# smilne36/ComponentFrameworks-smoothed-particle-hydrodynamics

Measured on AMD Instinct MI355X. Metric: particle-substeps/sec, higher is better.
Workload: dtype f32; 1 GPU; config3: 4194304 particles and a 128x128x128-cell grid per GPU (BASELINE.json configs[2]); particles=4194304, neighbor_kernel=k_sph_walk

## Files before the change

componentframeworks-smoothed-particle-hydrodynamics_amd/csrc/sph_engine.hip:

```cpp
#include <hip/hip_runtime.h>

#include <algorithm>
#include <chrono>
#include <cstdarg>
#include <cstdio>
#include <cstdlib>
#include <cstring>
#include <memory>
#include <mutex>
#include <set>
#include <string>
#include <thread>
#include <vector>

#include "../../include/sph_abi.h"
#include "sph_host.h"
#include "sph_kernels.h"
#include "sph_walk.h"
#include "sph_sample.h"
#include "sph_neighbors.h"
#include "sph_components.h"
#include "sph_knn.h"
#include "sph_aggregate.h"
#include "sph_conv.h"
// ... 177 lines not shown
    size_t cap = 0;
    int allocatedCells = 0;
    uint32_t idBase = 0;

    int optNeighbor = 3, optGridBuild = 0, optAos = 1, optTiming = 0, optGraph = 0;
    struct GraphEntry {
        uint64_t key = 0;
        std::vector<unsigned char> material;
        hipGraphExec_t exec = nullptr;
        int postCur = 0;
        bool postAos = false, postAcc = false;
        uint64_t lastUse = 0;
    };
    std::vector<GraphEntry> graphs;
    uint64_t graphClock = 0, graphLaunches = 0, graphCaptures = 0;

    SphParticle* d_aos = nullptr;
    float4* d_pos[2] = {nullptr, nullptr};
    float4* d_vel[2] = {nullptr, nullptr};
    float2* d_rp[2] = {nullptr, nullptr};
    float* d_foam[2] = {nullptr, nullptr};
    float4* d_acc = nullptr;
    int cur = 0;
    bool internalValid = false, aosValid = false, accValid = false;
    uint2* d_binKey = nullptr;
    uint32_t* d_order = nullptr;
    float4* d_stencil = nullptr;
    size_t stencilCount = 0;
    int32_t *d_llNext = nullptr, *d_llCell = nullptr, *d_llKey = nullptr;
    uint2* d_tmp = nullptr;
    uint32_t *d_cellCount = nullptr, *d_cellStart = nullptr, *d_blockSums = nullptr;
    int32_t* d_dbg = nullptr;
    size_t dbgCap = 0;
    bool slab = false;
    int z0 = 0, z1 = 0, hasLo = 0, hasHi = 0;
    size_t nSlots = 0;
    char* d_face[4] = {nullptr, nullptr, nullptr, nullptr};
    SlabSeen* h_seen = nullptr;
    hipEvent_t evCnt[4] = {nullptr, nullptr, nullptr, nullptr};
    bool cntValid[4] = {false, false, false, false};
    uint32_t exchangeNo = 0;
    sph::SlabMsg msgSend{}, msgRecv{};
    uint64_t sentBytes[2] = {0, 0};
    int calmHold = 0;
    uint32_t stepNo = 0;
    SphSlabIntent intent{};
    bool intentValid = false;
    uint32_t holdEvents = 0;
    int verifyMode = 1;
    double deadlineSec = 30.0;
    float lastDt = 0.0f;
    int tightMessages = 0;
    hipStream_t hstream = nullptr;
    hipEvent_t evIntent = nullptr;
    SlabPlans *d_intent = nullptr, *h_intent = nullptr;
    float handshakeMs = 0.0f;
    uint64_t handshakes = 0;
    bool stepPaused = false;
    float packGrid[8] = {0};
    bool packGridValid = false;
    hipEvent_t evX[5] = {nullptr, nullptr, nullptr, nullptr, nullptr};
    hipEvent_t evPassEnd = nullptr;
    uint32_t faceCap = 0;
    const void* faceAgreedWith = nullptr;
    SphFountain fountain{};
    SphRiver river{};
    std::vector<float> terrainHeights;
    float* d_terrain = nullptr;
    size_t terrainCap = 0;
    float4 *d_sPV = nullptr, *d_sOwn = nullptr;
    size_t sortedCap = 0;
    float4* d_shapeTab = nullptr;
    float shapeKey[8] = {-1.0f};
    sph::ShapeTab shapeTab{};
    hipStream_t xstream = nullptr;
    hipStream_t bstream = nullptr;
    hipEvent_t evBoundary = nullptr, evPacked = nullptr, evDone = nullptr, evSorted = nullptr, evInterior = nullptr;
    hipEvent_t peerDone[2] = {nullptr, nullptr};
    bool stepPending = false;
    bool slabOrderValid = false;
    float lastContainer[15] = {0};
    uint32_t* d_slabCnt = nullptr;
    int debugFlags = 0;
    unsigned long long* d_stats = nullptr;
    DevBuf<float4> d_sampleIn;
    DevBuf<SphSample> d_sampleOut;
    DevBuf<int32_t> d_slotIds;
    ScanScratch scanScratch;
    DevBuf<int32_t> d_nbIndices;
    DevBuf<uint32_t> d_nbCnt;
    DevBuf<long long> d_nbOffsets;
    SphNeighborInfo nbInfo{};
    bool nbIndexed = false;
    DevBuf<int32_t> d_ccIds, d_ccLabels, d_ccRoots;
    DevBuf<uint32_t> d_ccParent, d_ccMinId, d_ccFlag, d_ccWords;
    DevBuf<unsigned long long> d_ccStats;
    DevBuf<long long> d_ccOffsets;
    DevBuf<sph::CcRow> d_ccTable;
    SphComponentInfo ccInfo{};
    bool ccValid = false;
    int optCcVariant = 0;
    DevBuf<int32_t> d_knnIndices;
    DevBuf<float> d_knnDist2;
    DevBuf<uint32_t> d_knnCounts;
    DevBuf<unsigned long long> d_knnStats;
    SphKnnInfo knnInfo{};
    DevBuf<float4> d_rayIn, d_rayHits;
    DevBuf<unsigned long long> d_rayStats;
    DevBuf<uint2> d_rayBin;
    DevBuf<uint32_t> d_rayCount, d_rayStart, d_rayBlockSums, d_rayOrder;
    int optRaysVariant = 0;
    SphRaysInfo raysInfo{};
    bool raysValid = false;
    DevBuf<uint4> d_spanRows;
    DevBuf<unsigned long long> d_spanStats;
    int optRaySpansVariant = 0;
    SphRaySpansInfo spansInfo{};
    bool spansValid = false;
    int optKnnVariant = 0;
    DevBuf<float> d_aggStage, d_aggIn, d_aggOut;
    DevBuf<uint32_t> d_aggCnt;
    DevBuf<uint2> d_adjKey;
    DevBuf<uint32_t> d_adjCount, d_adjSums, d_adjStart, d_adjTmp, d_adjPerm, d_adjArg;
    DevBuf<float4> d_adjPts;
    DevBuf<float> d_adjIn;
    DevBuf<float> d_posStage;
    int optAggVariant = 0;
    DevBuf<sph::ShellRow> d_shRows;
    DevBuf<int32_t> d_shIds, d_shSlots;
    DevBuf<float4> d_shNrm;
    DevBuf<uint32_t> d_shFlagRow, d_shFlagSlot;
    DevBuf<unsigned long long> d_shStats;
    DevBuf<long long> d_shOffsets;
    SphShellInfo shellInfo{};
    DevBuf<sph::AnisoRow> d_anRows;
    DevBuf<float4> d_anSlots;
    DevBuf<unsigned long long> d_anStats;
    SphAnisoInfo anisoInfo{};
    int optShellTimed = 0;
    DevBuf<float> d_surfVol;
    DevBuf<uint16_t> d_surfCode;
    DevBuf<uint32_t> d_surfVOff, d_surfTris;
    DevBuf<uint2> d_surfTile;
    DevBuf<unsigned long long> d_surfTileOff;
    DevBuf<sph::SurfVertex> d_surfVerts;
    bool surfValid = false;
    uint32_t surfNumV = 0, surfNumT = 0;
    DevBuf<double> d_statSums;
    DevBuf<uint32_t> d_statPart, d_statHist;
    DevBuf<unsigned long long> d_statCell, d_statOut;

    float4* d_trRec = nullptr;
    uint32_t* d_trPerm = nullptr;
    float4* d_trRing = nullptr;
    uint32_t* d_trState = nullptr;
    uint2* d_trKey = nullptr;
    DevBuf<uint32_t> d_trCellCount, d_trCellStart, d_trBlockSums;
    size_t trM = 0, trCap = 0, trRingCap = 0;
    int trIntegrator = 0;
    uint32_t trK = 0, trS = 1;
    uint64_t trSteps = 0;
    uint64_t trSorted = 0;
    bool trOrdered = false;
    bool capturing = false;

    float4* d_dfPool = nullptr;
// ... 836 lines not shown
                          p.param_shapeAux[0], p.param_shapeAux[1], p.param_shapeAux[2], 1.0f};
    if (e->d_shapeTab && std::memcmp(key, e->shapeKey, sizeof(key)) == 0) return SPH_OK;
    int rc;
    if (!e->d_shapeTab && (rc = dev_alloc(&e->d_shapeTab, 128))) return rc;
    float pts[384], b0[3];
    const int cnt = shape_table(p, pts, b0);
    float4 host[128];
    for (int i = 0; i < cnt; ++i) host[i] = make_float4(pts[3 * i], pts[3 * i + 1], pts[3 * i + 2], 0.0f);
    if (cnt) {
        HIP_TRY(hipStreamSynchronize(e->stream));
        HIP_TRY(hipMemcpy(e->d_shapeTab, host, sizeof(float4) * (size_t)cnt, hipMemcpyHostToDevice));
    }
    e->shapeTab = sph::ShapeTab{e->d_shapeTab, cnt, b0[0], b0[1], b0[2]};
    std::memcpy(e->shapeKey, key, sizeof(key));
    return SPH_OK;
}

int dispatch_one(SphEngine* e, float overrideDt, bool boundaryFirst = false) {
    if (e->params.param_pause) { if (boundaryFirst) HIP_TRY(hipEventRecord(e->evBoundary, e->stream)); return SPH_OK; }
    int rc;
    if (e->trM && (rc = needs_sorted_copy(e, "tracers need"))) return rc;
    if (e->scK && (rc = needs_sorted_copy(e, "scalars need"))) return rc;
    if (e->dfC && (rc = needs_sorted_copy(e, "diffuse particles need"))) return rc;
    if (e->gtTab.count && (rc = needs_sorted_copy(e, "gates need"))) return rc;
    if (e->monCount && (rc = needs_sorted_copy(e, "monitors need"))) return rc;
    if ((rc = validate_params(e->params)) || (rc = couple_refused(e))) return rc;
    float cont[15];
    container_key(e->params, cont);
    const bool sameContainer = std::memcmp(cont, e->lastContainer, sizeof(cont)) == 0;
    const float dt = overrideDt > 0.0f ? overrideDt : e->params.param_timeStep;
    e->lastDt = dt;
    compute_grid_extents(e->params, e->grid);
    if ((rc = ensure_grid_buffers(e))) return rc;
    SimK k;
    make_simk(e->params, e->grid, dt, k);
    if (e->dfC && e->dfCrOn) {
        float radius = 0.0f;
        int stencil = 0;
        if (!diffuse_crest_args(e, k.cellSize, &radius, &stencil))
            return fail(SPH_ERR_STATE, "diffuse crest radius %g is above three cells (%g) of this grid", (double)radius, (double)(3.0f * k.cellSize));
    }
    if (e->slab) {
        if (e->z1 > e->grid.dims[2] || e->z0 < 0) return fail(SPH_ERR_STATE, "slab [%d,%d) outside the %d-layer grid", e->z0, e->z1, e->grid.dims[2]);
        k.gz = e->z1 - e->z0 + 2; k.numCells = k.gx * k.gy * k.gz; k.zoff = e->z0 - 1;
        if (e->optGridBuild != 1 && sameContainer) k.slabFlags = e->d_slabCnt + kSlabCntFlags;
    }
    if ((rc = import_state(e))) return rc;
    const int n = (int)(e->slab ? e->nSlots : e->n);
    StateIn in{e->d_pos[e->cur], e->d_vel[e->cur], e->d_rp[e->cur], e->d_foam[e->cur]};
    const int nx = e->cur ^ 1;
    if (k.obbDeferred && (rc = ensure_shape_table(e))) return rc;
    const bool fuseAos = !e->slab && e->optAos == 0 && e->aosValid && !k.obbDeferred && !e->obsK && !e->cpBuoy;
    StateOut out{e->d_pos[nx], e->d_vel[nx], e->d_rp[nx], e->d_foam[nx], e->d_acc, fuseAos ? e->d_aos : nullptr, e->idBase};
    if (e->optGridBuild == 1) {
        if (e->slab) return fail(SPH_ERR_STATE, "the linked-list variant is single-GPU only");
        if (!e->d_llNext) {
            if ((rc = dev_alloc(&e->d_llNext, e->cap)) || (rc = dev_alloc(&e->d_llCell, e->cap)) || (rc = dev_alloc(&e->d_llKey, e->cap))) return rc;
        }
        int32_t* cellHead = reinterpret_cast<int32_t*>(e->d_cellStart);
        {
            Timed t(e, SPH_K_SCAN);
            hipLaunchKernelGGL(k_ll_clear, dim3(blocks_for((size_t)k.numCells)), dim3(kBlock), 0, e->stream, cellHead, k.numCells);
        }
        if (n) {
            {
                Timed t(e, SPH_K_BIN);
                hipLaunchKernelGGL(k_ll_build, dim3(blocks_for(n)), dim3(kBlock), 0, e->stream, k, in.pos, cellHead, e->d_llNext, e->d_llCell, e->d_llKey, n);
            }
            Timed t(e, SPH_K_SPH);
            hipLaunchKernelGGL(k_sph_ll, dim3(blocks_for(n)), dim3(kBlock), 0, e->stream, k, in, out, cellHead, e->d_llNext, n);
        }
    } else {
    if ((rc = build_grid(e, k, true))) return rc;
    if (e->trM && (rc = tracers_advect(e, k, dt))) return rc;
    if (e->monCount && (rc = monitors_step(e, k, dt))) return rc;
    if (e->dfC && (rc = diffuse_step(e, k, dt, (uint32_t)n))) return rc;
    if (e->scK && (rc = scalars_step(e, k, dt))) return rc;
    if (n) {
        if (!e->d_sPV || e->sortedCap < (size_t)n) return fail(SPH_ERR_STATE, "sorted copy missing");
        const uint32_t* live = e->slab ? e->d_cellStart + k.numCells : nullptr;
        SortedIn S{e->d_sPV, e->d_sOwn};
        Timed t(e, SPH_K_SPH);
        if (e->optNeighbor >= 3 && (size_t)n < ((size_t)1 << 27)) {
            const dim3 grid(8 * ((blocks_for(n, 256) + 7) / 8));
            auto walk = [&](hipStream_t st, const uint32_t* lo, const uint32_t* hi, bool bothEnds = false) {
                const int dbg = (e->debugFlags & ~256) | (bothEnds ? 256 : 0);
                if (k.h2 <= 1.0f)
                    hipLaunchKernelGGL((k_sph_walk<SPH_WALK_MAXN, SPH_WALK_UNROLL, SPH_WALK_CAP, true>), grid, dim3(256), 0, st, k, S, in, out,
                                       e->d_order, e->d_cellStart, live, n, dbg, e->d_stats, lo, hi);
                else
                    hipLaunchKernelGGL((k_sph_walk<SPH_WALK_MAXN, SPH_WALK_UNROLL, SPH_WALK_CAP, false>), grid, dim3(256), 0, st, k, S, in, out,
                                       e->d_order, e->d_cellStart, live, n, dbg, e->d_stats, lo, hi);
            };
            const bool split = boundaryFirst && e->slab && k.gz > 2 * kSlabDepth && !k.obbDeferred && sameContainer;
            const bool timedStep = boundaryFirst && e->optTiming && e->evPassEnd;
            if (split) {
                const uint32_t* endLo = e->d_cellStart + kSlabDepth * (size_t)(k.gx * k.gy);
                const uint32_t* startHi = e->d_cellStart + (size_t)(k.gz - kSlabDepth) * (size_t)(k.gx * k.gy);
                HIP_TRY(hipEventRecord(e->evSorted, e->stream));
                walk(e->stream, endLo, startHi, true);
                HIP_TRY(hipEventRecord(e->evBoundary, e->stream));
                HIP_TRY(hipStreamWaitEvent(e->bstream, e->evSorted, 0));
                walk(e->bstream, endLo, startHi);
                HIP_TRY(hipEventRecord(e->evInterior, e->bstream));
                boundaryFirst = false;
                HIP_TRY(hipStreamWaitEvent(e->stream, e->evInterior, 0));
            } else {
                walk(e->stream, nullptr, nullptr);
            }
            if (timedStep) HIP_TRY(hipEventRecord(e->evPassEnd, e->stream));
        } else if (e->optNeighbor >= 2) {
            hipLaunchKernelGGL((k_sph_list<SPH_LIST_MAXN, SPH_LIST_UNROLL, SPH_LIST_CAP>), dim3(8 * ((blocks_for(n, SPH_LIST_BLOCK) + 7) / 8)), dim3(SPH_LIST_BLOCK), 0, e->stream, k, S, in, out,
                               e->d_order, e->d_cellStart, live, n, e->debugFlags, e->d_stats);
        } else {
            hipLaunchKernelGGL(k_sph_slow, dim3(blocks_for(n)), dim3(kBlock), 0, e->stream, k, S, in, out, e->d_order, e->d_cellStart, n);
        }
    }
    }
    if (n && k.obbDeferred) {
        Timed t(e, SPH_K_OTHER);
        const uint32_t* live = (e->slab && e->optGridBuild != 1) ? e->d_cellStart + k.numCells : nullptr;
        hipLaunchKernelGGL(k_obb_ext, dim3(blocks_for(n)), dim3(kBlock), 0, e->stream, k, e->shapeTab, out.pos, out.vel, live, n,
                           (e->slab && e->optGridBuild != 1) ? (const float4*)e->d_sOwn : (const float4*)nullptr);
    }
    if (e->obsK && (rc = obstacles_step(e, out.pos, out.vel, n, dt))) return rc;
    if (e->scK && (e->cpBuoy || e->cpTab.nSrc) && (rc = couple_step(e, out.pos, out.vel, n, dt))) return rc;
    if (e->gtTab.count && (rc = gates_step(e, out.pos, out.vel, n, dt))) return rc;
    const bool riverOn = e->river.riverMode && !e->terrainHeights.empty();
    if (riverOn) {
        if (e->slab) return fail(SPH_ERR_STATE, "riverMode on a z-slab engine: recycled particles jump across slabs (single-GPU engines only)");
        if (n) {
            const SphParams& p = e->params;
            const SphRiver& r = e->river;
            RiverK rk{r.terrainW, r.terrainH, r.terrainWorldMinX, r.terrainWorldMinZ, r.terrainWorldSizeX, r.terrainWorldSizeZ,
                      0.02f, 1.0f - 0.05f, p.param_boxCenter[0], r.riverAmp, r.riverFreq, r.riverPhase, r.riverChannelWidth,
                      80.0f, p.param_timeStep, r.riverSinkY, r.riverSinkZMax, r.riverEmitterPos[0], r.riverEmitterPos[1], r.riverEmitterPos[2],
                      r.riverEmitterVel[0], r.riverEmitterVel[1], r.riverEmitterVel[2], r.riverEmitterRadius,
                      r.riverSinkZMax - r.riverEmitterPos[2], p.param_restDensity};
            Timed t(e, SPH_K_OTHER);
            hipLaunchKernelGGL(k_river, dim3(blocks_for(n)), dim3(kBlock), 0, e->stream, rk, e->d_terrain, out.pos, out.vel, out.rp,
                               fuseAos ? (float4*)nullptr : e->d_acc, fuseAos ? e->d_aos : (SphParticle*)nullptr, e->d_aos, e->idBase, n);
        }
    }
    if (e->fountain.fountainMode && !e->river.riverMode) {
        if (e->slab) return fail(SPH_ERR_STATE, "fountainMode on a z-slab engine: recycled particles jump across slabs (single-GPU engines only)");
        if (n) {
            float half[3];
            effective_half(e->params, half);
            const SphParams& p = e->params;
            const SphFountain& f = e->fountain;
            FountainK fk{p.param_boxCenter[0] + f.fountainOffset[0], p.param_boxCenter[1] + f.fountainOffset[1],
                         p.param_boxCenter[2] + f.fountainOffset[2], f.fountainRadius, f.fountainSpread, f.fountainJetSpeedLive,
                         (p.param_boxCenter[1] - half[1]) + f.fountainDrainLevel, std::fmin(1.0f, f.fountainDrainPerSec * dt),
                         p.param_restDensity, f.fountainSeed * 747796405u};
            Timed t(e, SPH_K_OTHER);
            const uint32_t* live = (e->slab && e->optGridBuild != 1) ? e->d_cellStart + k.numCells : nullptr;
            hipLaunchKernelGGL(k_fountain, dim3(blocks_for(n)), dim3(kBlock), 0, e->stream, fk, out.pos, out.vel, out.rp,
                               fuseAos ? (float4*)nullptr : e->d_acc, fuseAos ? e->d_aos : (SphParticle*)nullptr, e->idBase, live, n);
        }
        e->fountain.fountainSeed++;
    }
    HIP_TRY(hipGetLastError());
    if (boundaryFirst) HIP_TRY(hipEventRecord(e->evBoundary, e->stream));
    e->cur = nx;
    e->accValid = !fuseAos;
    e->aosValid = fuseAos;
    if (e->slab) {
        const bool sorted = e->optGridBuild != 1 && n > 0;
        if (!sorted) HIP_TRY(hipMemcpyAsync(e->d_slabCnt + kSlabCntLive, e->d_cellStart + k.numCells, sizeof(uint32_t), hipMemcpyDeviceToDevice, e->stream));
        if (!sameContainer) slab_hold(e);
        std::memcpy(e->lastContainer, cont, sizeof(cont));
        e->slabOrderValid = sorted && sameContainer;
        return SPH_OK;
    }
    if (e->optAos == 0 && !e->aosValid) return writeback(e);
// ... 9 lines not shown
    sph::compute_grid_extents(e->params, e->grid);
    SlabGeom g;
    g.gminz = e->grid.gridMin[2]; g.cellSize = e->grid.cellSize; g.gzGlobal = e->grid.dims[2];
    g.z0 = e->z0; g.z1 = e->z1; g.hasLo = e->hasLo; g.hasHi = e->hasHi;
    return g;
}

int slab_engine(const SphEngine* e, bool needFaces = false) {
    if (!e) return fail(SPH_ERR_ARG, "null engine");
    if (needFaces) return e->slab && e->d_face[0] ? SPH_OK : fail(SPH_ERR_STATE, "slab engine with face buffers required");
    return e->slab ? SPH_OK : fail(SPH_ERR_STATE, "not a slab engine");
}

int slab_flags_error(const SphEngine* e, uint32_t flags, uint32_t nLo, uint32_t nHi) {
    if (flags & SPH_SLAB_FLAG_SEND_OVERFLOW) return fail(SPH_ERR_CAPACITY, "halo send buffer overflowed (%u / %u records for a capacity of %u)", nLo, nHi, e->faceCap);
    if (flags & SPH_SLAB_FLAG_SLOT_OVERFLOW) return fail(SPH_ERR_CAPACITY, "slab capacity %zu exceeded while appending halo records", e->cap);
    if (flags & SPH_SLAB_FLAG_BAD_HEADER) return fail(SPH_ERR_HIP, "a received halo message did not start with a valid header (magic / count): failed or garbled receive");
    if (flags & SPH_SLAB_FLAG_TRUNCATED) return fail(SPH_ERR_CAPACITY, "a neighbour rank had more halo records than its message could carry (face capacity %u)", e->faceCap);
    if (flags & SPH_SLAB_FLAG_SIZE_MISMATCH) return fail(SPH_ERR_STATE, "the two ends of a link sized an exchange's messages differently (a received header names other message sizes than this engine received): "
                                                "the ranks' call sequences differ");
    return SPH_OK;
}

template <class K>
int launch_impulse(SphEngine* e, const K& kk) {
    int rc;
    if ((rc = import_state(e))) return rc;
    const size_t nw = e->slab ? e->nSlots : e->n;
    if (e->slab) slab_hold(e);
    if (nw) {
        Timed t(e, SPH_K_IMPULSE);
        hipLaunchKernelGGL((k_impulse<K>), dim3(blocks_for(nw)), dim3(kBlock), 0, e->stream, kk, e->d_pos[e->cur], e->d_vel[e->cur],
                           (e->aosValid && !e->slab) ? e->d_aos : nullptr, e->idBase, (int)nw);
    }
    HIP_TRY(hipGetLastError());
    return SPH_OK;
}
}

extern "C" {

int sph_abi_version(void) { return SPH_ABI_VERSION; }
const char* sph_last_error(void) { return g_err.c_str(); }

int sph_params_default(SphParams* out) {
    if (!out) return fail(SPH_ERR_ARG, "null params");
    sph::params_default(*out);
    return SPH_OK;
}
int sph_rotation_mat3(const float eulerDeg[3], float outM[9]) {
    if (!eulerDeg || !outM) return fail(SPH_ERR_ARG, "null argument");
    sph::rotation_mat3(eulerDeg, outM);
    return SPH_OK;
}
int sph_effective_half(const SphParams* params, float outHalf[3]) {
    if (!params || !outHalf) return fail(SPH_ERR_ARG, "null argument");
    sph::effective_half(*params, outHalf);
    return SPH_OK;
}
int sph_compute_grid_extents(const SphParams* params, SphGridInfo* out) {
    if (!params || !out) return fail(SPH_ERR_ARG, "null argument");
    sph::compute_grid_extents(*params, *out);
    return SPH_OK;
}
int sph_spawn_particles(const SphParams* params, size_t nRequested, uint32_t seed, SphParticle* out, size_t* nOut, float* massOut) {
    if (!params || !out || !nOut || !massOut) return fail(SPH_ERR_ARG, "null argument");
    std::vector<SphParticle> v;
    float m;
    sph::spawn_particles(*params, nRequested, seed, v, m);
    std::memcpy(out, v.data(), v.size() * sizeof(SphParticle));
    *nOut = v.size();
    *massOut = m;
    return SPH_OK;
}

static int create_common(SphEngine** out, const SphParams* params, void* stream, SphEngine** made) {
    if (!out || !params) return fail(SPH_ERR_ARG, "null argument");
    *out = nullptr;
    int rc;
    if ((rc = validate_params(*params))) return rc;
    int ndev = 0;
    HIP_TRY(hipGetDeviceCount(&ndev));
    if (ndev <= 0) return fail(SPH_ERR_HIP, "no HIP device: this engine has no CPU fallback");
    SphEngine* e = new SphEngine();
    volumes_unbind_all(e);
    sph_fountain_default(&e->fountain);
    sph_river_default(&e->river);
    e->params = *params;
    if (stream) { e->stream = (hipStream_t)stream; e->ownStream = false; }
    else {
        hipError_t er = hipStreamCreateWithFlags(&e->stream, hipStreamNonBlocking);
        if (er != hipSuccess) { delete e; return fail(SPH_ERR_HIP, "hipStreamCreate failed: %s", hipGetErrorString(er)); }
        e->ownStream = true;
    }
    *made = e;
    { std::lock_guard<std::mutex> lk(g_enginesMutex); g_engines.insert(e); }
    return SPH_OK;
}

int sph_create(SphEngine** out, size_t nRequested, const SphParams* params, uint32_t seed, void* stream) {
    SphEngine* e = nullptr;
    int rc = create_common(out, params, stream, &e);
    if (rc) return rc;
    std::vector<SphParticle> v;
    float m;
    sph::spawn_particles(e->params, nRequested, seed, v, m);
    e->params.param_mass = m;
    sph::compute_grid_extents(e->params, e->grid);
    if ((rc = set_particles(e, v.data(), v.size())) || (rc = ensure_grid_buffers(e))) { sph_destroy(e); return rc; }
    *out = e;
    return SPH_OK;
}

int sph_create_from_particles(SphEngine** out, const SphParticle* particles, size_t n, const SphParams* params, void* stream) {
    if (!particles && n) return fail(SPH_ERR_ARG, "null particles");
    SphEngine* e = nullptr;
    int rc = create_common(out, params, stream, &e);
    if (rc) return rc;
    sph::compute_grid_extents(e->params, e->grid);
    if ((rc = set_particles(e, particles, n)) || (rc = ensure_grid_buffers(e))) { sph_destroy(e); return rc; }
    *out = e;
    return SPH_OK;
}

int sph_destroy(SphEngine* e) {
    if (!e) return SPH_OK;
    if (e->stream) (void)hipStreamSynchronize(e->stream);
    if (e->xstream) (void)hipStreamSynchronize(e->xstream);
    if (e->bstream) (void)hipStreamSynchronize(e->bstream);
    free_particle_buffers(e);
    free_grid_buffers(e);
    dev_free(e->d_dbg);
    dev_free(e->d_stencil);
    dev_free(e->d_terrain);
    dev_free(e->d_stats);
    sample_free(e);
    neighbors_free(e);
    components_free(e);
    knn_free(e);
    rays_free(e);
    shell_free(e);
    aniso_free(e);
    aggregate_free(e);
    surface_free(e);
    stats_free(e);
    tracers_free(e);
    diffuse_free(e);
    scalars_free(e);
    gates_free(e);
    monitors_free(e);
    obstacles_free(e);
    volumes_free(e);
    e->d_stateAcc.release();
    for (auto& ev : e->evLive) { (void)hipEventDestroy(ev.a); (void)hipEventDestroy(ev.b); }
    for (auto& ev : e->evPool) { (void)hipEventDestroy(ev.first); (void)hipEventDestroy(ev.second); }
    if (e->xstream) { (void)hipStreamSynchronize(e->xstream); (void)hipStreamDestroy(e->xstream); }
    if (e->bstream) { (void)hipStreamSynchronize(e->bstream); (void)hipStreamDestroy(e->bstream); }
    {
        std::lock_guard<std::mutex> lk(g_enginesMutex);
        for (SphEngine* o : g_engines)
            for (auto& pd : o->peerDone) if (pd && pd == e->evDone) pd = nullptr;
        g_engines.erase(e);
    }
    for (hipEvent_t ev : {e->evBoundary, e->evPacked, e->evDone, e->evSorted, e->evInterior, e->evPassEnd}) if (ev) (void)hipEventDestroy(ev);
    for (hipEvent_t ev : e->evX) if (ev) (void)hipEventDestroy(ev);
    for (hipEvent_t ev : e->evCnt) if (ev) (void)hipEventDestroy(ev);
    if (e->h_seen) (void)hipHostFree(e->h_seen);
// ... 6458 lines not shown
```

componentframeworks-smoothed-particle-hydrodynamics_amd/csrc/sph_pass.h:

```cpp
#pragma once
#include <type_traits>

#include "sph_kernels.h"

namespace sph {

struct SortedIn {
    const float4* __restrict__ pv;
    const float4* __restrict__ own;
    __device__ __forceinline__ float4 P(uint32_t q) const { return pv[2u * q]; }
    __device__ __forceinline__ float4 V(uint32_t q) const { return pv[2u * q + 1u]; }
};

typedef float v4f __attribute__((ext_vector_type(4)));

template <bool STREAM = false>
__device__ __forceinline__ void store_fields(const SimK& k, const StateOut& out, int s, uint32_t flags, uint32_t id, float px, float py,
                                             float pz, float vx, float vy, float vz, float ax, float ay, float az, float rho, float prs,
                                             float foamOut, int czEntry) {
    if (!(flags & F_GHOSTNZ)) obb_apply(k, px, py, pz, vx, vy, vz);
    slab_check_layer_move(k, czEntry, pz);
    if constexpr (!STREAM) {
        out.pos[s] = make_float4(px, py, pz, bitsf(flags));
        out.vel[s] = make_float4(vx, vy, vz, bitsf(id));
        out.rp[s] = make_float2(rho, prs);
        out.foam[s] = foamOut;
    } else {
        __builtin_nontemporal_store(v4f{px, py, pz, bitsf(flags)}, reinterpret_cast<v4f*>(&out.pos[s]));
        __builtin_nontemporal_store(v4f{vx, vy, vz, bitsf(id)}, reinterpret_cast<v4f*>(&out.vel[s]));
        __builtin_nontemporal_store(v2f{rho, prs}, reinterpret_cast<v2f*>(&out.rp[s]));
        __builtin_nontemporal_store(foamOut, &out.foam[s]);
    }
    if (out.aos) aos_write_fluid(out.aos, id - out.idBase, px, py, pz, vx, vy, vz, ax, ay, az, rho, prs, foamOut);
    else if constexpr (!STREAM) out.acc[s] = make_float4(ax, ay, az, 0.0f);
    else __builtin_nontemporal_store(v4f{ax, ay, az, 0.0f}, reinterpret_cast<v4f*>(&out.acc[s]));
}

__device__ __forceinline__ bool special_slot(const SimK& k, const SortedIn& S, const StateIn& in, const StateOut& out,
                                             const uint32_t* __restrict__ order, int s, const float4& P, const float4& V, const float4& O) {
    const uint32_t flags = fbits(O.z), id = fbits(O.w);
    if (flags & F_HALO) { out.pos[s] = make_float4(P.x, P.y, P.z, O.z); return true; }
    if (flags & F_GHOST1) {
        float gvx = V.x, gvy = V.y, gvz = V.z, grho = in.rp[order[s]].x, gprs = V.w;
        if (!(flags & F_INACTIVE)) { gvx = gvy = gvz = 0.0f; grho = k.rho0; gprs = 0.0f; }
        out.pos[s] = make_float4(P.x, P.y, P.z, O.z);
        out.vel[s] = make_float4(gvx, gvy, gvz, O.w);
        out.rp[s] = make_float2(grho, gprs);
        out.foam[s] = O.y;
        if (out.aos) { if (!(flags & F_INACTIVE)) aos_write_active_ghost(out.aos, id - out.idBase, k.rho0); }
        else out.acc[s] = make_float4(0.0f, 0.0f, 0.0f, 0.0f);
        return true;
    }
    return false;
}

__device__ __forceinline__ void sph_slow_one(const SimK& k, const SortedIn& S, const StateIn& in, const StateOut& out,
                                          const uint32_t* __restrict__ order, const uint32_t* __restrict__ cellStart, int s) {
    const float4 P = S.P(s), V = S.V(s), O = S.own[s];
    if (special_slot(k, S, in, out, order, s, P, V, O)) return;
    const uint32_t cb = fbits(O.x);
    const int cx = (int)(cb & 1023u), cy = (int)((cb >> 10) & 1023u), cz = (int)(cb >> 20);
    Own o;
    own_reset(o);
    o.px = P.x; o.py = P.y; o.pz = P.z; o.vx = V.x; o.vy = V.y; o.vz = V.z; o.rho = 0.0f; o.prs = 0.0f;
    const int xlo = max(cx - 1, 0), xhi = min(cx + 1, k.gx - 1);
    auto rows = [&](auto&& f) {
        for (int r = 0; r < 9; ++r) {
            const int nz = cz + r / 3 - 1, ny = cy + r % 3 - 1;
            if (nz < 0 || nz >= k.gz || ny < 0 || ny >= k.gy) continue;
            const int rowBase = (nz * k.gy + ny) * k.gx;
            const uint32_t qs = cellStart[rowBase + xlo], qe = cellStart[rowBase + xhi + 1];
            for (uint32_t q = qs; q < qe; ++q) f(q);
        }
    };
    rows([&](uint32_t q) { const float4 J = S.P(q); pair_density(k, o, J.x, J.y, J.z, (int32_t)-1); });
    finish_density(k, o);
    rows([&](uint32_t q) {
        const float4 J = S.P(q), JV = S.V(q);
        pair_force(k, o, J.x, J.y, J.z, JV.x, JV.y, JV.z, JV.w, J.w, (int32_t)((int)q != s ? -1 : 0));
    });
    integrate(k, o);
    rows([&](uint32_t q) {
        const float4 J = S.P(q), JV = S.V(q);
        pair_xsph(k, o, J.x, J.y, J.z, JV.x, JV.y, JV.z, J.w, (int32_t)((int)q != s ? -1 : 0));
    });
    const float foamOut = finish_particle(k, o, O.y);
    store_fields(k, out, s, fbits(O.z), fbits(O.w), o.px, o.py, o.pz, o.vx, o.vy, o.vz, o.ax, o.ay, o.az, o.rho, o.prs, foamOut, cz);
}

__global__ __launch_bounds__(kBlock) void k_sph_slow(SimK k, SortedIn S, StateIn in, StateOut out, const uint32_t* __restrict__ order,
                                                     const uint32_t* __restrict__ cellStart, int n) {
    const int s = blockIdx.x * kBlock + threadIdx.x;
    if (s >= n || (uint32_t)s >= cellStart[k.numCells]) return;
    sph_slow_one(k, S, in, out, order, cellStart, s);
}

#ifndef SPH_LIST_MAXN
#define SPH_LIST_MAXN 47
#endif
#ifndef SPH_LIST_CAP
#define SPH_LIST_CAP 96
#endif
#ifndef SPH_LIST_UNROLL
#define SPH_LIST_UNROLL 3
#endif
#ifndef SPH_LIST_WAVES
#define SPH_LIST_WAVES 5
#endif
#ifndef SPH_LIST_BLOCK
#define SPH_LIST_BLOCK 256
#endif
#ifndef SPH_LIST_EPS
#define SPH_LIST_EPS 0.06f
#endif
#ifndef SPH_LIST_LISTU
#define SPH_LIST_LISTU 4
#endif
#ifndef SPH_LIST_CHUNKG
#define SPH_LIST_CHUNKG 4
#endif

template <int MAXN, int UNROLL, int CAP>
__global__ __launch_bounds__(SPH_LIST_BLOCK, SPH_LIST_WAVES) void k_sph_list(SimK k, SortedIn S, StateIn in, StateOut out, const uint32_t* __restrict__ order,
                                                     const uint32_t* __restrict__ cellStart, const uint32_t* __restrict__ liveCount, int n, int dbg,
                                                     unsigned long long* __restrict__ stats) {
    constexpr int kB = SPH_LIST_BLOCK;
    __shared__ uint16_t nl[MAXN + UNROLL][kB];
    __shared__ uint32_t rowA[kB / 64][12];
    __shared__ float4 stage[kB / 64][CAP];
    const int tid = threadIdx.x;
    const int lane = tid & 63, wv = tid >> 6;
    const int bound = liveCount ? min(n, (int)*liveCount) : n;
    const int nBlocks = (bound + kB - 1) / kB, perXcd = (nBlocks + 7) >> 3;
// ... 189 lines not shown
```

componentframeworks-smoothed-particle-hydrodynamics_amd/csrc/sph_walk.h:

```cpp
#pragma once
#include "sph_pass.h"

namespace sph {

#ifndef SPH_WALK_MAXN
#define SPH_WALK_MAXN 41
#endif
#ifndef SPH_WALK_CAP
#define SPH_WALK_CAP 144
#endif
#ifndef SPH_WALK_UNROLL
#define SPH_WALK_UNROLL 3
#endif
#ifndef SPH_WALK_WAVES
#define SPH_WALK_WAVES 5
#endif
#ifndef SPH_WALK_EPS
#define SPH_WALK_EPS 0.04f
#endif

typedef unsigned int v4u32 __attribute__((ext_vector_type(4)));

__device__ __forceinline__ float4 buf_load4(__amdgpu_buffer_rsrc_t r, uint32_t byteOff) {
    const v4u32 v = __builtin_amdgcn_raw_buffer_load_b128(r, (int)byteOff, 0, 0);
    return make_float4(bitsf(v.x), bitsf(v.y), bitsf(v.z), bitsf(v.w));
}

__device__ __forceinline__ void pair_force_other(const SimK& k, Own& o, const float4& J, const float4& JV) {
    const float dx = o.px - J.x, dy = o.py - J.y, dz = o.pz - J.z;
    const float r2 = dot3(dx, dy, dz, dx, dy, dz);
    const int32_t in = (int32_t)fbits(r2 - k.h2) >> 31;
    const float ie = bitsf(fbits(J.w) & (uint32_t)in);
    const float rinv = t_rsqrt(fmaxf(r2, SPH_TINY));
    const float r = r2 * rinv;
    const float hr = k.h - r;
    const float sr = (k.spikyC * (hr * hr)) * rinv;
    const float gx = sr * dx, gy = sr * dy, gz = sr * dz;
    const float mor = k.mass * ie;
    const float pterm = ((o.prs + JV.w) * k.negHalfMass) * ie;
    const float ml = mor * (k.viscC * hr);
    o.fPx = fmaf(gx, pterm, o.fPx); o.fPy = fmaf(gy, pterm, o.fPy); o.fPz = fmaf(gz, pterm, o.fPz);
    o.fVx = fmaf(JV.x - o.vx, ml, o.fVx); o.fVy = fmaf(JV.y - o.vy, ml, o.fVy); o.fVz = fmaf(JV.z - o.vz, ml, o.fVz);
    o.gCx = fmaf(mor, gx, o.gCx); o.gCy = fmaf(mor, gy, o.gCy); o.gCz = fmaf(mor, gz, o.gCz);
    o.lapC = o.lapC + ml;
}
template <bool SMALLH>
__device__ __forceinline__ void pair_xsph_other(const SimK& k, Own& o, const float4& J, const float4& JV) {
    const float dx = o.px - J.x, dy = o.py - J.y, dz = o.pz - J.z;
    const float r2 = dot3(dx, dy, dz, dx, dy, dz);
    const float t0 = SMALLH ? __builtin_amdgcn_fmed3f(k.h2 - r2, 0.0f, 1.0f) : fmaxf(k.h2 - r2, 0.0f);
    const int32_t has = (int32_t)(0u - fbits(J.w)) >> 31;
    const float t = bitsf(fbits(t0) & (uint32_t)has);
    const float w3 = (t * t) * t;
    const float wm = w3 * (k.mass * J.w);
    o.xsx = fmaf(JV.x - o.vx, wm, o.xsx); o.xsy = fmaf(JV.y - o.vy, wm, o.xsy); o.xsz = fmaf(JV.z - o.vz, wm, o.xsz);
    o.norm = o.norm + w3;
}

template <int MAXN, int UNROLL, int CAP, bool SMALLH>
__global__ __launch_bounds__(256, SPH_WALK_WAVES) void k_sph_walk(SimK k, SortedIn S, StateIn in, StateOut out, const uint32_t* __restrict__ order,
                                                                  const uint32_t* __restrict__ cellStart, const uint32_t* __restrict__ liveCount, int n,
                                                                  int dbg, unsigned long long* __restrict__ stats, const uint32_t* __restrict__ rangeLo,
                                                                  const uint32_t* __restrict__ rangeHi) {
    constexpr int kB = 256;
    constexpr uint32_t kRowBytes = kB * 2;
    static_assert(kRowBytes == 512, "the cursor advance reads bit 9 of (sign >> 22)");
    constexpr int kSpare = UNROLL > 2 ? UNROLL : 2;
    __shared__ uint16_t nl[MAXN + kSpare][kB];
    __shared__ uint32_t rowA[kB / 64][16];
    __shared__ float4 stage[kB / 64][CAP];
    static_assert(CAP <= 192, "the window is staged with three loads per lane, and a window offset has 8 bits in an entry");
    const int tid = threadIdx.x;
    const int lane = tid & 63, wv = tid >> 6;
    const int boundAll = liveCount ? min(n, (int)*liveCount) : n;
    const bool ends = (dbg & 256) != 0;
    int first = (rangeLo && !ends) ? min((int)*rangeLo, boundAll) : 0;
    int bound = rangeHi ? min((int)*rangeHi, boundAll) : boundAll;
    int vb;
    if (!ends) {
        const int nBlocks = (max(bound - first, 0) + kB - 1) / kB, perXcd = (nBlocks + 7) >> 3;
        vb = ((int)blockIdx.x & 7) * perXcd + ((int)blockIdx.x >> 3);
        if (((int)blockIdx.x >> 3) >= perXcd || vb >= nBlocks) return;
    } else {
        const int endLo = min((int)*rangeLo, boundAll), startHi = max(bound, endLo);
        const int nLo = (endLo + kB - 1) / kB, nHi = (max(boundAll - startHi, 0) + kB - 1) / kB, perXcd = (nLo + nHi + 7) >> 3;
        vb = ((int)blockIdx.x & 7) * perXcd + ((int)blockIdx.x >> 3);
        if (((int)blockIdx.x >> 3) >= perXcd || vb >= nLo + nHi) return;
        if (vb < nLo) { first = 0; bound = endLo; } else { first = startHi; bound = boundAll; vb -= nLo; }
    }
    const int sRaw = first + vb * kB + tid;
    bool live = sRaw < bound;
    const int s = live ? sRaw : max(bound - 1, 0);
    const float4 P = S.P(s), V = S.V(s), O = S.own[s];
    if (live && special_slot(k, S, in, out, order, s, P, V, O)) live = false;
    Own o;
    own_reset(o);
    o.px = P.x; o.py = P.y; o.pz = P.z; o.vx = V.x; o.vy = V.y; o.vz = V.z; o.rho = 0.0f; o.prs = 0.0f;
    const uint32_t cb = fbits(O.x);
    const int cx = (int)(cb & 1023u), cy = (int)((cb >> 10) & 1023u), cz = (int)(cb >> 20);
    const int xlo = max(cx - 1, 0), xhi = min(cx + 1, k.gx - 1);
    const __amdgpu_buffer_rsrc_t bufPV = __builtin_amdgcn_make_buffer_rsrc((void*)S.pv, 0, (int)((uint32_t)n * 32u), 0x00020000);
    const float eps = SPH_WALK_EPS * k.h;
    const float hp = k.h + eps;
    const float qx = fmaf(0.995f * fmaf(k.gravx, k.dt, o.vx), k.dt, o.px), qy = fmaf(0.995f * fmaf(k.gravy, k.dt, o.vy), k.dt, o.py),
                qz = fmaf(0.995f * fmaf(k.gravz, k.dt, o.vz), k.dt, o.pz);
    const float mvx = qx - o.px, mvy = qy - o.py, mvz = qz - o.pz;
    const float ex = mvx + mvx, ey = mvy + mvy, ez = mvz + mvz;
    const float mm = dot3(mvx, mvy, mvz, mvx, mvy, mvz);
    const float c0 = mm - (hp * hp) * 1.0001f;
    constexpr float kBig = 0x1p40f;
    uint32_t qs[9], qe[9];
#pragma unroll
    for (int r = 0; r < 9; ++r) {
        const int nz = cz + r / 3 - 1, ny = cy + r % 3 - 1;
        const bool in = live && nz >= 0 && nz < k.gz && ny >= 0 && ny < k.gy;
        const int rowBase = in ? (nz * k.gy + ny) * k.gx : 0;
        const uint32_t a = cellStart[rowBase + xlo], b = cellStart[rowBase + xhi + 1];
        qs[r] = in ? a : 0u; qe[r] = in ? b : 0u;
    }
    bool listOk = !(dbg & 1) && !(mm > 256.0f * k.h2);
    uint32_t cur = (uint32_t)tid * 2u;
    const uint32_t curEnd = (uint32_t)tid * 2u + (uint32_t)MAXN * kRowBytes;
    const uint32_t adv = live ? kRowBytes : 0u;
    char* const nlBytes = reinterpret_cast<char*>(&nl[0][0]);
    uint32_t eSelf = 0xffffffffu;
    auto density = [&](const float4& J, float& r2, float& t) {
        const float dx = o.px - J.x, dy = o.py - J.y, dz = o.pz - J.z;
        r2 = dot3(dx, dy, dz, dx, dy, dz);
        t = SMALLH ? __builtin_amdgcn_fmed3f(k.h2 - r2, 0.0f, 1.0f) : fmaxf(k.h2 - r2, 0.0f);
        o.dsum = fmaf(t * t, t, o.dsum);
        return fmaf(ez, dz, fmaf(ey, dy, fmaf(ex, dx, r2 + c0)));
    };
    auto visit = [&](const float4& J, uint32_t e, bool selfRow) {
        float r2, t;
        const float w = density(J, r2, t);
        float sg = fmaf(-kBig, t, w);
        if (selfRow) sg = (e == eSelf) ? 1.0f : sg;
        *reinterpret_cast<uint16_t*>(nlBytes + cur) = (uint16_t)e;
        cur += (fbits(sg) >> 22) & adv;
    };
    unsigned long long mneN = 0ull;
    uint32_t aN = 0u, bN = 0u;
    bool stagedN = false;
    float4 pre0 = make_float4(0.0f, 0.0f, 0.0f, 0.0f), pre1 = pre0, pre2 = pre0;
    const uint32_t laneOff32 = (uint32_t)lane * 32u;
    auto plan = [&](uint32_t q0, uint32_t q1) {
        const bool ne = q1 > q0;
        mneN = __ballot(ne);
        aN = bN = 0u; stagedN = false;
        if (mneN == 0ull) return;
        const int lf = __ffsll((long long)mneN) - 1, ll = 63 - __clzll((long long)mneN);
        const uint32_t A = (uint32_t)__builtin_amdgcn_readlane((int)q0, lf);
        const uint32_t B = (uint32_t)__builtin_amdgcn_readlane((int)q1, ll);
        aN = A; bN = B;
        stagedN = (B - A) <= (uint32_t)CAP && !(dbg & 4);
        if (stagedN) {
            const __amdgpu_buffer_rsrc_t rw = __builtin_amdgcn_make_buffer_rsrc((void*)(S.pv + 2u * (size_t)A), 0, (int)((B - A) * 32u), 0x00020000);
            pre0 = buf_load4(rw, laneOff32);
            if (CAP > 64) pre1 = buf_load4(rw, laneOff32 + 2048u);
            if (CAP > 128) pre2 = buf_load4(rw, laneOff32 + 4096u);
        }
    };
    int nRows = 0, nUnstaged = 0;
    plan(qs[0], qe[0]);
#pragma unroll
    for (int r = 0; r < 9; ++r) {
        const uint32_t q0 = qs[r], q1 = qe[r];
        const bool ne = q1 > q0;
        const unsigned long long mne = mneN;
        const uint32_t A = aN, B = bN;
        const bool staged = stagedN;
        const bool selfRow = (r == 4);
        if (mne != 0ull && staged) {
            const uint32_t e0 = ((uint32_t)r << 12) | ((uint32_t)lane << 4);
            stage[wv][lane] = make_float4(pre0.x, pre0.y, pre0.z, bitsf(e0));
            if (CAP > 64 && (CAP >= 128 || lane < CAP - 64)) stage[wv][lane + 64] = make_float4(pre1.x, pre1.y, pre1.z, bitsf(e0 + (64u << 4)));
            if (CAP > 128 && lane < CAP - 128) stage[wv][lane + 128] = make_float4(pre2.x, pre2.y, pre2.z, bitsf(e0 + (128u << 4)));
        }
        if (r < 8) plan(qs[r + 1], qe[r + 1]);
        if (mne == 0ull) continue;
        nRows += 1; nUnstaged += staged ? 0 : 1;
        const uint32_t len = q1 - q0;
        if (lane == 0) rowA[wv][r] = A * 32u;
        if (B - A > 255u) listOk = false;
        const uint32_t off = ne ? q0 - A : 0u;
        if (selfRow) eSelf = (4u << 12) | ((((uint32_t)s - A) << 4) & 0xff0u);
        if (staged) {
            __builtin_amdgcn_wave_barrier();
            const float4* __restrict__ wp = &stage[wv][off];
            uint32_t m = 0;
            for (; m + UNROLL <= len; m += UNROLL) {
                float4 J[UNROLL];
#pragma unroll
                for (int u = 0; u < UNROLL; ++u) J[u] = wp[m + (uint32_t)u];
                cur = min(cur, curEnd);
#pragma unroll
                for (int u = 0; u < UNROLL; ++u) visit(J[u], fbits(J[u].w), selfRow);
            }
            for (; m < len; ++m) {
                const float4 J = wp[m];
                cur = min(cur, curEnd);
                visit(J, fbits(J.w), selfRow);
            }
            __builtin_amdgcn_wave_barrier();
        } else {
            uint32_t e = ((uint32_t)r << 12) | ((off << 4) & 0xff0u);
            uint32_t m = 0;
            for (; m + UNROLL <= len; m += UNROLL) {
                float4 J[UNROLL];
#pragma unroll
                for (int u = 0; u < UNROLL; ++u) J[u] = S.P(q0 + m + (uint32_t)u);
                cur = min(cur, curEnd);
#pragma unroll
                for (int u = 0; u < UNROLL; ++u) visit(J[u], e + 16u * (uint32_t)u, selfRow);
                e += 16u * UNROLL;
            }
            for (; m < len; ++m, e += 16u) {
                const float4 J = S.P(q0 + m);
                cur = min(cur, curEnd);
                visit(J, e, selfRow);
            }
        }
    }
    __builtin_amdgcn_wave_barrier();
    listOk = (listOk && cur < curEnd) || !live;
    finish_density(k, o);


    const char* const rowBytes = reinterpret_cast<const char*>(&rowA[tid >> 6][0]);
    auto fetch = [&](uint32_t at, float4& J, float4& JV) {
        const uint32_t ent = *reinterpret_cast<const uint16_t*>(nlBytes + at);
        const uint32_t base = *reinterpret_cast<const uint32_t*>(rowBytes + ((ent >> 10) & 0x3cu));
        const uint32_t qb = base + ((ent & 0xff0u) << 1);
        J = buf_load4(bufPV, qb); JV = buf_load4(bufPV, qb + 16u);
    };
    auto listed = [&](auto&& f) {
        const uint32_t end = cur;
        uint32_t at = (uint32_t)tid * 2u;
        float4 J0, V0, J1, V1, J2, V2, J3, V3;
        J0 = V0 = J1 = V1 = J2 = V2 = J3 = V3 = make_float4(0.0f, 0.0f, 0.0f, 0.0f);
        if (at < end) fetch(at, J0, V0);
        if (at + kRowBytes < end) fetch(at + kRowBytes, J1, V1);
        while (at < end) {
            if (at + 2u * kRowBytes < end) fetch(at + 2u * kRowBytes, J2, V2);
            f(J0, V0);
            if (at + 3u * kRowBytes < end) fetch(at + 3u * kRowBytes, J3, V3);
            if (at + kRowBytes < end) f(J1, V1);
            at += 2u * kRowBytes;
            if (!(at < end)) break;
            if (at + 2u * kRowBytes < end) fetch(at + 2u * kRowBytes, J0, V0);
            f(J2, V2);
            if (at + 3u * kRowBytes < end) fetch(at + 3u * kRowBytes, J1, V1);
            if (at + kRowBytes < end) f(J3, V3);
            at += 2u * kRowBytes;
        }
    };
    static_assert(kSpare >= 2, "the walks read up to two rows past the last entry");
    auto plain = [&](auto&& f) {
        for (int r = 0; r < 9; ++r) {
            const int nz = cz + r / 3 - 1, ny = cy + r % 3 - 1;
            if (nz < 0 || nz >= k.gz || ny < 0 || ny >= k.gy) continue;
            const int rowBase = (nz * k.gy + ny) * k.gx;
            const uint32_t a = cellStart[rowBase + xlo], b = cellStart[rowBase + xhi + 1];
            auto within = [&](const float4& J) { const float dx = o.px - J.x, dy = o.py - J.y, dz = o.pz - J.z; return dot3(dx, dy, dz, dx, dy, dz) < k.h2; };
            uint32_t q = a;
            for (; q + 2u <= b; q += 2u) {
                const float4 J0 = S.P(q), V0 = S.V(q), J1 = S.P(q + 1u), V1 = S.V(q + 1u);
                if (__any(within(J0))) f(J0, V0, (int32_t)((int)q != s ? -1 : 0));
                if (__any(within(J1))) f(J1, V1, (int32_t)((int)(q + 1u) != s ? -1 : 0));
            }
            if (q < b) { const float4 J = S.P(q); if (__any(within(J))) f(J, S.V(q), (int32_t)((int)q != s ? -1 : 0)); }
        }
    };
    auto force_at = [&](const float4& J, const float4& JV) { pair_force_other(k, o, J, JV); };
    auto xsph_at = [&](const float4& J, const float4& JV) { pair_xsph_other<SMALLH>(k, o, J, JV); };
    auto force_plain = [&](const float4& J, const float4& JV, int32_t ok) { pair_force(k, o, J.x, J.y, J.z, JV.x, JV.y, JV.z, JV.w, J.w, ok); };
    auto xsph_plain = [&](const float4& J, const float4& JV, int32_t ok) { pair_xsph(k, o, J.x, J.y, J.z, JV.x, JV.y, JV.z, J.w, ok); };
    if (listOk) listed(force_at); else plain(force_plain);
    integrate(k, o);
    const float mx = o.px - qx, my = o.py - qy, mz = o.pz - qz;
    const float lim = 0.98f * eps;
    const bool near = (dot3(mx, my, mz, mx, my, mz) <= lim * lim && !(dbg & 2)) || !live;
    if (listOk && near) listed(xsph_at); else plain(xsph_plain);
    const float foamOut = finish_particle(k, o, O.y);
    if (live) store_fields<true>(k, out, s, fbits(O.z), fbits(O.w), o.px, o.py, o.pz, o.vx, o.vy, o.vz, o.ax, o.ay, o.az, o.rho, o.prs, foamOut, cz);
    if (dbg & 8) {
        const unsigned long long slowT = (unsigned long long)__popcll(__ballot(live && !(listOk && near)));
        unsigned long long ents = (unsigned long long)((live && listOk) ? (cur - (uint32_t)tid * 2u) / kRowBytes : 0u);
        for (int d = 32; d >= 1; d >>= 1) ents += (unsigned long long)__shfl_xor((int)ents, d, 64);
        const unsigned long long ovf = (unsigned long long)__popcll(__ballot(live && !listOk)), far = (unsigned long long)__popcll(__ballot(live && listOk && !near));
        if (lane == 0) { atomicAdd(&stats[0], (unsigned long long)nUnstaged); atomicAdd(&stats[3], (unsigned long long)nRows); atomicAdd(&stats[1], slowT); atomicAdd(&stats[2], ents & 0xffffffffull); atomicAdd(&stats[4], 64ull); atomicAdd(&stats[5], ovf); atomicAdd(&stats[6], far); atomicAdd(&stats[7], slowT ? 1ull : 0ull); }
    }
}

}
```

Before: 1.421 billion particle-substeps/s.

## Make SPH walk kernel persistent with per-XCD grid-stride tiles and prefetch

The walk kernel launch is changed from one block per 256 particles to a persistent grid sized to compute units times waves per CU, a multiple of eight. Each block loops over tiles in an XCD-contiguous range, and each wave skips empty 64-particle slices. The next tile's ownership record is prefetched during the current tile's force phase. Kernel arguments are packed into a struct reread from the kernarg segment each iteration, and asm barriers keep tid and zero in VGPRs, presumably to limit scalar register pressure. This saves block launch and LDS setup costs and overlaps one load, but it risks load imbalance across tiles and possible register or scheduling regressions.

After: 1.230 billion particle-substeps/s. -13.4%, worse.

```diff
diff --git a/componentframeworks-smoothed-particle-hydrodynamics_amd/csrc/sph_engine.hip b/componentframeworks-smoothed-particle-hydrodynamics_amd/csrc/sph_engine.hip
--- a/componentframeworks-smoothed-particle-hydrodynamics_amd/csrc/sph_engine.hip
+++ b/componentframeworks-smoothed-particle-hydrodynamics_amd/csrc/sph_engine.hip
@@ -283,6 +283,7 @@
     float lastContainer[15] = {0};
     uint32_t* d_slabCnt = nullptr;
     int debugFlags = 0;
+    int walkBlocks = 0;
     unsigned long long* d_stats = nullptr;
     DevBuf<float4> d_sampleIn;
     DevBuf<SphSample> d_sampleOut;
@@ -1285,15 +1286,14 @@
         SortedIn S{e->d_sPV, e->d_sOwn};
         Timed t(e, SPH_K_SPH);
         if (e->optNeighbor >= 3 && (size_t)n < ((size_t)1 << 27)) {
-            const dim3 grid(8 * ((blocks_for(n, 256) + 7) / 8));
+            const dim3 grid(e->walkBlocks);
             auto walk = [&](hipStream_t st, const uint32_t* lo, const uint32_t* hi, bool bothEnds = false) {
                 const int dbg = (e->debugFlags & ~256) | (bothEnds ? 256 : 0);
+                const WalkArgs a{k, S, in, out, e->d_order, e->d_cellStart, live, n, dbg, e->d_stats, lo, hi};
                 if (k.h2 <= 1.0f)
-                    hipLaunchKernelGGL((k_sph_walk<SPH_WALK_MAXN, SPH_WALK_UNROLL, SPH_WALK_CAP, true>), grid, dim3(256), 0, st, k, S, in, out,
-                                       e->d_order, e->d_cellStart, live, n, dbg, e->d_stats, lo, hi);
+                    hipLaunchKernelGGL((k_sph_walk<SPH_WALK_MAXN, SPH_WALK_UNROLL, SPH_WALK_CAP, true>), grid, dim3(256), 0, st, a);
                 else
-                    hipLaunchKernelGGL((k_sph_walk<SPH_WALK_MAXN, SPH_WALK_UNROLL, SPH_WALK_CAP, false>), grid, dim3(256), 0, st, k, S, in, out,
-                                       e->d_order, e->d_cellStart, live, n, dbg, e->d_stats, lo, hi);
+                    hipLaunchKernelGGL((k_sph_walk<SPH_WALK_MAXN, SPH_WALK_UNROLL, SPH_WALK_CAP, false>), grid, dim3(256), 0, st, a);
             };
             const bool split = boundaryFirst && e->slab && k.gz > 2 * kSlabDepth && !k.obbDeferred && sameContainer;
             const bool timedStep = boundaryFirst && e->optTiming && e->evPassEnd;
@@ -1469,7 +1469,12 @@
     int ndev = 0;
     HIP_TRY(hipGetDeviceCount(&ndev));
     if (ndev <= 0) return fail(SPH_ERR_HIP, "no HIP device: this engine has no CPU fallback");
+    int dev = 0, cus = 0;
+    HIP_TRY(hipGetDevice(&dev));
+    HIP_TRY(hipDeviceGetAttribute(&cus, hipDeviceAttributeMultiprocessorCount, dev));
+    if (cus < 8) return fail(SPH_ERR_HIP, "device %d reports %d compute units: the SPH pass maps its blocks to 8 XCDs", dev, cus);
     SphEngine* e = new SphEngine();
+    e->walkBlocks = 8 * (cus / 8) * SPH_WALK_WAVES;
     volumes_unbind_all(e);
     sph_fountain_default(&e->fountain);
     sph_river_default(&e->river);
diff --git a/componentframeworks-smoothed-particle-hydrodynamics_amd/csrc/sph_pass.h b/componentframeworks-smoothed-particle-hydrodynamics_amd/csrc/sph_pass.h
--- a/componentframeworks-smoothed-particle-hydrodynamics_amd/csrc/sph_pass.h
+++ b/componentframeworks-smoothed-particle-hydrodynamics_amd/csrc/sph_pass.h
@@ -37,7 +37,8 @@
 }
 
 __device__ __forceinline__ bool special_slot(const SimK& k, const SortedIn& S, const StateIn& in, const StateOut& out,
-                                             const uint32_t* __restrict__ order, int s, const float4& P, const float4& V, const float4& O) {
+                                             const uint32_t* __restrict__ order, int s, const float4& P, const float4& V, const float4& O,
+                                             float zero = 0.0f) {
     const uint32_t flags = fbits(O.z), id = fbits(O.w);
     if (flags & F_HALO) { out.pos[s] = make_float4(P.x, P.y, P.z, O.z); return true; }
     if (flags & F_GHOST1) {
@@ -48,7 +49,7 @@
         out.rp[s] = make_float2(grho, gprs);
         out.foam[s] = O.y;
         if (out.aos) { if (!(flags & F_INACTIVE)) aos_write_active_ghost(out.aos, id - out.idBase, k.rho0); }
-        else out.acc[s] = make_float4(0.0f, 0.0f, 0.0f, 0.0f);
+        else out.acc[s] = make_float4(zero, zero, zero, zero);
         return true;
     }
     return false;
diff --git a/componentframeworks-smoothed-particle-hydrodynamics_amd/csrc/sph_walk.h b/componentframeworks-smoothed-particle-hydrodynamics_amd/csrc/sph_walk.h
--- a/componentframeworks-smoothed-particle-hydrodynamics_amd/csrc/sph_walk.h
+++ b/componentframeworks-smoothed-particle-hydrodynamics_amd/csrc/sph_walk.h
@@ -57,42 +57,30 @@
     o.norm = o.norm + w3;
 }
 
+struct WalkArgs {
+    SimK k; SortedIn S; StateIn in; StateOut out;
+    const uint32_t* order; const uint32_t* cellStart;
+    const uint32_t* liveCount;
+    int n, dbg;
+    unsigned long long* stats;
+    const uint32_t* rangeLo; const uint32_t* rangeHi;
+};
+
 template <int MAXN, int UNROLL, int CAP, bool SMALLH>
-__global__ __launch_bounds__(256, SPH_WALK_WAVES) void k_sph_walk(SimK k, SortedIn S, StateIn in, StateOut out, const uint32_t* __restrict__ order,
-                                                                  const uint32_t* __restrict__ cellStart, const uint32_t* __restrict__ liveCount, int n,
-                                                                  int dbg, unsigned long long* __restrict__ stats, const uint32_t* __restrict__ rangeLo,
-                                                                  const uint32_t* __restrict__ rangeHi) {
+__device__ __forceinline__ void walk_tile(const SimK& k, const SortedIn& S, const StateIn& in, const StateOut& out, const uint32_t* __restrict__ order,
+                                          const uint32_t* __restrict__ cellStart, int n, int dbg, unsigned long long* __restrict__ stats,
+                                          uint16_t (*nl)[256], uint32_t (*rowA)[16], float4 (*stage)[CAP],
+                                          int tid, float zero, int s0, int bound, float4& Oio, int s0Next, int boundNext) {
     constexpr int kB = 256;
     constexpr uint32_t kRowBytes = kB * 2;
     static_assert(kRowBytes == 512, "the cursor advance reads bit 9 of (sign >> 22)");
     constexpr int kSpare = UNROLL > 2 ? UNROLL : 2;
-    __shared__ uint16_t nl[MAXN + kSpare][kB];
-    __shared__ uint32_t rowA[kB / 64][16];
-    __shared__ float4 stage[kB / 64][CAP];
-    static_assert(CAP <= 192, "the window is staged with three loads per lane, and a window offset has 8 bits in an entry");
-    const int tid = threadIdx.x;
     const int lane = tid & 63, wv = tid >> 6;
-    const int boundAll = liveCount ? min(n, (int)*liveCount) : n;
-    const bool ends = (dbg & 256) != 0;
-    int first = (rangeLo && !ends) ? min((int)*rangeLo, boundAll) : 0;
-    int bound = rangeHi ? min((int)*rangeHi, boundAll) : boundAll;
-    int vb;
-    if (!ends) {
-        const int nBlocks = (max(bound - first, 0) + kB - 1) / kB, perXcd = (nBlocks + 7) >> 3;
-        vb = ((int)blockIdx.x & 7) * perXcd + ((int)blockIdx.x >> 3);
-        if (((int)blockIdx.x >> 3) >= perXcd || vb >= nBlocks) return;
-    } else {
-        const int endLo = min((int)*rangeLo, boundAll), startHi = max(bound, endLo);
-        const int nLo = (endLo + kB - 1) / kB, nHi = (max(boundAll - startHi, 0) + kB - 1) / kB, perXcd = (nLo + nHi + 7) >> 3;
-        vb = ((int)blockIdx.x & 7) * perXcd + ((int)blockIdx.x >> 3);
-        if (((int)blockIdx.x >> 3) >= perXcd || vb >= nLo + nHi) return;
-        if (vb < nLo) { first = 0; bound = endLo; } else { first = startHi; bound = boundAll; vb -= nLo; }
-    }
-    const int sRaw = first + vb * kB + tid;
-    bool live = sRaw < bound;
-    const int s = live ? sRaw : max(bound - 1, 0);
-    const float4 P = S.P(s), V = S.V(s), O = S.own[s];
-    if (live && special_slot(k, S, in, out, order, s, P, V, O)) live = false;
+    const float4 zero4 = make_float4(zero, zero, zero, zero);
+    bool live = s0 + lane < bound;
+    const int s = live ? s0 + lane : bound - 1;
+    const float4 P = S.P(s), V = S.V(s), O = Oio;
+    if (live && special_slot(k, S, in, out, order, s, P, V, O, zero)) live = false;
     Own o;
     own_reset(o);
     o.px = P.x; o.py = P.y; o.pz = P.z; o.vx = V.x; o.vy = V.y; o.vz = V.z; o.rho = 0.0f; o.prs = 0.0f;
@@ -142,7 +130,7 @@
     unsigned long long mneN = 0ull;
     uint32_t aN = 0u, bN = 0u;
     bool stagedN = false;
-    float4 pre0 = make_float4(0.0f, 0.0f, 0.0f, 0.0f), pre1 = pre0, pre2 = pre0;
+    float4 pre0 = zero4, pre1 = pre0, pre2 = pre0;
     const uint32_t laneOff32 = (uint32_t)lane * 32u;
     auto plan = [&](uint32_t q0, uint32_t q1) {
         const bool ne = q1 > q0;
@@ -225,7 +213,7 @@
     __builtin_amdgcn_wave_barrier();
     listOk = (listOk && cur < curEnd) || !live;
     finish_density(k, o);
-
+    if (s0Next >= 0) Oio = S.own[min(s0Next + lane, boundNext - 1)];
 
     const char* const rowBytes = reinterpret_cast<const char*>(&rowA[tid >> 6][0]);
     auto fetch = [&](uint32_t at, float4& J, float4& JV) {
@@ -238,7 +226,7 @@
         const uint32_t end = cur;
         uint32_t at = (uint32_t)tid * 2u;
         float4 J0, V0, J1, V1, J2, V2, J3, V3;
-        J0 = V0 = J1 = V1 = J2 = V2 = J3 = V3 = make_float4(0.0f, 0.0f, 0.0f, 0.0f);
+        J0 = V0 = J1 = V1 = J2 = V2 = J3 = V3 = zero4;
         if (at < end) fetch(at, J0, V0);
         if (at + kRowBytes < end) fetch(at + kRowBytes, J1, V1);
         while (at < end) {
@@ -293,4 +281,59 @@
     }
 }
 
-}
+template <int MAXN, int UNROLL, int CAP, bool SMALLH>
+__global__ __launch_bounds__(256, SPH_WALK_WAVES) void k_sph_walk(WalkArgs args) {
+    constexpr int kB = 256;
+    constexpr int kSpare = UNROLL > 2 ? UNROLL : 2;
+    __shared__ uint16_t nl[MAXN + kSpare][kB];
+    __shared__ uint32_t rowA[kB / 64][16];
+    __shared__ float4 stage[kB / 64][CAP];
+    static_assert(CAP <= 192, "the window is staged with three loads per lane, and a window offset has 8 bits in an entry");
+    const int wvU = __builtin_amdgcn_readfirstlane((int)threadIdx.x >> 6);
+    const int boundAll = args.liveCount ? min(args.n, (int)*args.liveCount) : args.n;
+    const bool ends = (args.dbg & 256) != 0;
+    int firstA, boundA, firstB = 0, boundB = 0;
+    if (!ends) {
+        firstA = args.rangeLo ? min((int)*args.rangeLo, boundAll) : 0;
+        boundA = args.rangeHi ? min((int)*args.rangeHi, boundAll) : boundAll;
+    } else {
+        const int bound = args.rangeHi ? min((int)*args.rangeHi, boundAll) : boundAll;
+        firstA = 0; boundA = min((int)*args.rangeLo, boundAll);
+        firstB = max(bound, boundA); boundB = boundAll;
+    }
+    const int nA = (max(boundA - firstA, 0) + kB - 1) / kB, nTiles = nA + (max(boundB - firstB, 0) + kB - 1) / kB;
+    const int perXcd = (nTiles + 7) >> 3, tile0 = ((int)blockIdx.x & 7) * perXcd, stride = (int)gridDim.x >> 3;
+    auto tile_at = [&](int t, int& s0, int& bound) {
+        const int vb = tile0 + t;
+        if (t >= perXcd || vb >= nTiles) return false;
+        const bool inA = vb < nA;
+        s0 = (inA ? firstA + vb * kB : firstB + (vb - nA) * kB) + wvU * 64;
+        bound = inA ? boundA : boundB;
+        return true;
+    };
+    auto advance = [&](int& t, int& s0, int& bound) {
+        for (t += stride; tile_at(t, s0, bound); t += stride) {
+            if (s0 < bound) return true;
+            if ((args.dbg & 8) && ((int)threadIdx.x & 63) == 0) atomicAdd(&args.stats[4], 64ull);
+        }
+        return false;
+    };
+    int t = ((int)blockIdx.x >> 3) - stride, s0, bound;
+    if (!advance(t, s0, bound)) return;
+    float4 O = args.S.own[min(s0 + ((int)threadIdx.x & 63), bound - 1)];
+    for (;;) {
+        int tn = t, s0n, boundn;
+        if (!advance(tn, s0n, boundn)) s0n = -1;
+        const __attribute__((address_space(4))) WalkArgs* ap = (const __attribute__((address_space(4))) WalkArgs*)__builtin_amdgcn_kernarg_segment_ptr();
+        asm volatile("" : "+s"(ap));
+        const WalkArgs& a = *(const WalkArgs*)ap;
+        int tid = (int)threadIdx.x;
+        float zero = 0.0f;
+        asm volatile("" : "+v"(tid), "+v"(zero));
+        walk_tile<MAXN, UNROLL, CAP, SMALLH>(a.k, a.S, a.in, a.out, a.order, a.cellStart, a.n, a.dbg, a.stats, nl, rowA, stage, tid, zero, s0, bound, O, s0n, boundn);
+        if (s0n < 0) break;
+        t = tn; s0 = s0n; bound = boundn;
+    }
+}
+
+}
```
